# wjqkkky/TTS

Measured on AMD Instinct MI355X. Metric: mel-frames/s (Tacotron2-DDC + MB-MelGAN end-to-end), higher is better.
Workload: dtype f32; 1 GPU; C2: Tacotron2-DDC (r_init=7, r=2, sigmoid attn) + MB-MelGAN [8,4,2]x4, 32 LJ-length utterances per GPU; global_batch=32, r=2, parallelism=replicas x1

## Files before the change

tts_amd/csrc/api_core.hip:

```cpp
#include "host.h"
#include "split16.h"
#include "switches.h"

#include <cmath>
#include <cstring>
#include <memory>

static thread_local std::string g_err;
void tts_set_error(const std::string& m) { g_err = m; }

namespace ttsh {

__global__ void put_rows_kernel(int* dst, RowInts r, int n) {
  if ((int)threadIdx.x < n) dst[threadIdx.x] = r.v[threadIdx.x];
}

const int* put_rows(int* dst, const int32_t* h, int n, hipStream_t s) {
  for (int o = 0; o < n; o += BMAX) {
    const int m = std::min(BMAX, n - o);
    put_rows_kernel<<<1, BMAX, 0, s>>>(dst + o, row_ints(h + o, m), m);
    HIP_OK(hipGetLastError());
  }
  return dst;
}
// ... 155 lines not shown
  a.resid = c.resid;
  a.rb = c.rb;
  a.rc = c.rc;
  a.rt = c.rt;
  a.resid_rows = c.resid_rows;
  a.aux = c.aux;
  a.auxb = c.auxb;
  a.max_q = c.max_q;
  a.B = c.B;
  a.merged_u = c.merged_u;
  TTS_CHECK(!c.merged_u || (c.oflow && L.W16.p), "phase-merged ConvTranspose runs on split-f16 weights only");
  if (c.oflow && L.W16.p && c.nsrc == 1 && (c.s[0].sc != 1 || c.s[0].st % 4 == 0)) {
    a.W16 = L.W16.p;
    a.w16_phase_stride = L.w16_stride;
    a.oflow = c.oflow;
    launch_conv_x3(a, st);
    return;
  }
  launch_conv(a, L.tile, st);
}

void enter(tts_ctx* c, void* stream, bool join_voc) {
  if (c->sv_live && join_voc) {
    HIP_OK(hipStreamWaitEvent(c->s, c->ev_sv, 0));
    c->sv_live = false;
  }
  if (hipStreamQuery((hipStream_t)stream) == hipSuccess) return;
  (void)hipGetLastError();
  HIP_OK(hipEventRecord(c->ev_in, (hipStream_t)stream));
  HIP_OK(hipStreamWaitEvent(c->s, c->ev_in, 0));
}
// ... 151 lines not shown
```

tts_amd/csrc/api_ge2e.hip:

```cpp
#include "host.h"
#include "gsync.h"
#include "split16.h"
#include "switches.h"

#include <cmath>

using namespace ttsh;

namespace {

__global__ void pad_channels_kernel(const float* __restrict__ x, int D, int Dp, long n_rows, float* __restrict__ y) {
  for (long i = (long)blockIdx.x * blockDim.x + threadIdx.x; i < n_rows * Dp; i += (long)gridDim.x * blockDim.x) {
    const long r = i / Dp;
    const int c = (int)(i - r * Dp);
    y[i] = c < D ? x[r * D + c] : 0.f;
  }
}

__global__ __launch_bounds__(256) void ge2e_final_kernel(const float* __restrict__ src, long sb, int width,
                                                         const int* lens, int T_max, const float* __restrict__ W,
                                                         const float* __restrict__ bias, int P,
                                                         float* __restrict__ out) {
  __shared__ float v[1024], red[4];
  const int b = blockIdx.x, tid = threadIdx.x;
// ... 112 lines not shown
  hipStream_t s = c->s;
  const int H = G.H;
  ensure<float>(W.x, (size_t)B * T_max * G.in_pad);
  ensure<int>(W.lens, 64);
  ensure<float>(W.g, (size_t)B * T_max * 4 * H);
  ensure<float>(W.o, (size_t)B * T_max * H);
  ensure<float>(W.p, (size_t)B * T_max * G.proj);
  ensure<unsigned>(W.bar, BAR_WORDS);
  ensure<float>(W.hbuf, (size_t)2 * 64 * H);
  const int* dl = put_rows(W.lens, h_lens, B, s);
  pad_channels_kernel<<<1024, 256, 0, s>>>(d_x, G.in_dim, G.in_pad, (long)B * T_max, W.x.f());
  HIP_OK(hipGetLastError());
  const float* in = W.x.f();
  int din = G.in_pad;
  auto gates = [&](int l) {
    run_conv(G.gin[l], conv_call(c, dl, B, T_max).in(in, btc(T_max, din), din).to(W.g.f(), btc(T_max, 4 * H)), s);
  };
  auto project = [&](int l) {
    run_conv(G.proj_l[l], conv_call(c, dl, B, T_max).in(W.o.f(), btc(T_max, H), H).to(W.p.f(), btc(T_max, G.proj)), s);
  };
  const bool pipe_env = sw::ge2e_pipe();
  bool piped = false;
  if (pipe_env && c->gemm_x3 && G.pipe_ok && B <= 16) {
    gates(0);
    const uint16_t* w16[4] = {nullptr, nullptr, nullptr, nullptr};
    const float* bias[4] = {nullptr, nullptr, nullptr, nullptr};
    for (int l = 0; l < G.nl; ++l) {
      w16[l] = l == 0 ? G.whh16[0].h() : G.wpipe[l].h();
      bias[l] = l == 0 ? nullptr : G.bpipe[l].f();
    }
    piped = launch_ge2e_pipe(w16, bias, G.nl, W.g.f(), dl, T_max, B, W.hbuf.f(), reinterpret_cast<unsigned*>(W.bar.p),
                             W.o.f(), s);
    if (piped && G.with_proj) project(G.nl - 1);
  }
// ... 53 lines not shown
```

tts_amd/csrc/api_glow.hip:

```cpp
#include "host.h"

#include <cmath>
#include <cstdlib>

using namespace ttsh;

namespace {

std::pair<std::vector<float>, std::vector<float>> interleave_halves(const std::vector<float>& w,
                                                                           const std::vector<float>& b, int half,
                                                                           int rowlen) {
  std::vector<float> wo(w.size()), bo(b.size());
  for (int r = 0; r < 2 * half; ++r) {
    const int src = (r & 1) ? half + r / 2 : r / 2;
    std::copy(w.begin() + (size_t)src * rowlen, w.begin() + (size_t)(src + 1) * rowlen, wo.begin() + (size_t)r * rowlen);
    bo[r] = b[src];
  }
  return {wo, bo};
}

void glow_finalize(tts_ctx* c, int num_chars, int enc_layers, int flows, int wn_layers) {
  auto& G = c->glow;
  const auto& h = c->glow_host;
  G.ready = false;
// ... 284 lines not shown
    ensure<float>(W.g, (size_t)B * G.c_pad);
    ensure<float>(W.gcond, (size_t)B * NC);
    if (!W.ones.p) {
      std::vector<int> one(64, 1);
      W.ones.upload(one);
    }
    launch_glow_speaker(put_rows(W.spk, h_spk, B, s), G.emb_g.f(), G.c_in, G.c_pad, W.g.f(), B, s);
    run_conv(G.cond, conv_call(c, W.ones.i(), B, 1).in(W.g.f(), bct(G.c_pad, 1), G.c_pad).to(W.gcond.f(), bct(NC, 1)), s);
  }
  float* x = W.xa.f();
  float* x2 = W.xb.f();
  launch_glow_embed(d_ids, T, G.emb.f(), G.num_chars, H, dl, x, B, s);
  auto conv = [&](const ConvLayer& L, const float* in, int cin, float* out, int cout, int epi,
                  const float* resid = nullptr) {
    ConvCall cc = conv_call(c, dl, B, T).in(in, bct(cin, T), cin).to(out, bct(cout, T)).add(resid, bct(cout, T));
    cc.epi = epi;
    run_conv(L, cc, s);
  };
  if (G.tdsep || G.tfm) {
    float* h0 = W.h2.f();
    float* h1 = W.hdp.f();
    conv(G.pre_conv[0], x, H, h0, H, 0);
    launch_ln(h0, (long)H * T, H, G.pre_g[0].f(), G.pre_b[0].f(), dl, B, T, s, true);
    conv(G.pre_conv[1], h0, H, h1, H, 0);
    launch_ln(h1, (long)H * T, H, G.pre_g[1].f(), G.pre_b[1].f(), dl, B, T, s, true);
    conv(G.pre_conv[2], h1, H, h0, H, 0);
    launch_ln(h0, (long)H * T, H, G.pre_g[2].f(), G.pre_b[2].f(), dl, B, T, s, true);
    conv(G.pre_proj, h0, H, x2, H, 0, x);
    std::swap(x, x2);
    for (int i = 0; i < (G.tfm ? G.enc_layers : 0); ++i) {
// ... 33 lines not shown
  conv(G.dp2, W.hdp.f(), F, W.h2.f(), F, 1);
  launch_ln(W.h2.f(), (long)F * T, F, G.dp_g2.f(), G.dp_b2.f(), dl, B, T, s);
  conv(G.dp_proj, W.h2.f(), F, W.logw.f(), 1, 0);
  launch_glow_durations(W.logw.f(), T, dl, length_scale, W.cum.f(), W.ylens.i(), W.wceil.f(), B, s);
  HIP_OK(hipMemcpyAsync(h_ylens, W.ylens.p, B * 4, hipMemcpyDeviceToHost, s));
  HIP_OK(hipStreamSynchronize(s));
  int mx = 1;
  W.h_ylens.assign(h_ylens, h_ylens + B);
  for (int b = 0; b < B; ++b) mx = std::max(mx, (int)h_ylens[b]);
  W.Ty = mx;
}

struct FlowConvs {
  tts_ctx* c;
  const int* kl;
  int B, K;
  void conv(const ConvLayer& L, const float* in, int in_rows, float* out, int out_rows, const float* resid, int epi,
            int resid_rows = 0, const float* aux = nullptr) const {
    const auto& G = c->glow;
    ConvCall cc = conv_call(c, kl, B, K).in(in, bct(in_rows, K), L.Cin).to(out, bct(out_rows, K));
    cc.add(resid, bct(out_rows, K));
    cc.epi = epi;
    cc.resid_rows = resid_rows;
    cc.aux = aux;
    cc.auxb = (long)G.flows * G.wn_layers * 2 * G.H;
    run_conv(L, cc, c->s);
  }
  float* wn(int k, const float* x) const {
    const auto& G = c->glow;
    auto& W = c->glws;
    const int H = G.H;
    float* hid = W.whs.f();
    float* skip = W.whs.f() + (size_t)H * K;
    conv(G.start[k], x, 2 * G.C, hid, 2 * H, nullptr, 0);
    for (int i = 0; i < G.wn_layers; ++i) {
      const int li = k * G.wn_layers + i;
// ... 15 lines not shown
  const int K1 = std::max(K, 1);
  ensure<float>(W.z, (size_t)B * C * Ty);
  ensure<float>(W.sq, (size_t)B * C2 * K1);
  ensure<float>(W.sq2, (size_t)B * C2 * K1);
  ensure<float>(W.whs, (size_t)B * 2 * H * K1);
  ensure<float>(W.wacts, (size_t)B * H * K1);
  launch_glow_expand(W.om.f(), C, Tx, W.lens.i(), W.cum.f(), W.ylens.i(), Ty, d_noise, noise_scale, d_ymean, W.z.f(),
                     d_attn, B, s);
  HIP_OK(hipMemcpyAsync(d_logw, W.logw.p, (size_t)B * Tx * 4, hipMemcpyDeviceToDevice, s));
  HIP_OK(hipMemsetAsync(d_y, 0, (size_t)B * C * 2 * K * 4, s));
  if (K == 0) return;
  RowInts hk{};
  for (int b = 0; b < B; ++b) hk.v[b] = W.h_ylens[b] / 2;
  const int* kl = put_rows(W.klens, hk.v, B, s);
  launch_glow_squeeze(W.z.f(), C, Ty, W.ylens.i(), W.sq.f(), K, B, s);
  const FlowConvs fc{c, kl, B, K};
  float* x = W.sq.f();
  float* x2 = W.sq2.f();
  for (int k = G.flows - 1; k >= 0; --k) {
    const float* skip = fc.wn(k, x);
    fc.conv(G.end[k], skip, 2 * H, x2, C2, x, 5, 0, G.invtab[k].f());
    std::swap(x, x2);
  }
  launch_glow_unsqueeze(x, C2, K, W.ylens.i(), d_y, 2 * K, B, s);
  HIP_OK(hipStreamSynchronize(s));
}

void glow_search(tts_ctx* c, const float* d_logp, const int* xl, const int* yl, int max_xlen, int B, int Tx, int Ty) {
  auto& W = c->glws;
  ensure<unsigned long long>(W.masbits, (size_t)B * glow_mas_bits_words(Tx, Ty));
  ensure<int>(W.xof, (size_t)B * Ty);
// ... 26 lines not shown
  ensure<int>(W.aylens, 64);
  ensure<int>(W.aklens, 64);
  ensure<float>(W.sq, (size_t)B * C2 * K);
  ensure<float>(W.sq2, (size_t)B * C2 * K);
  ensure<float>(W.eo, (size_t)B * C2 * K);
  ensure<float>(W.whs, (size_t)B * 2 * H * K);
  ensure<float>(W.wacts, (size_t)B * H * K);
  ensure<double>(W.ldpart, (size_t)G.flows * B * tiles);
  if (!d_logp) {
    ensure<float>(W.logp, (size_t)B * Tx * Te);
    d_logp = W.logp.f();
  }
  const int* yl = put_rows(W.aylens, ye2.v, B, s);
  const int* kl = put_rows(W.aklens, ke.v, B, s);
  launch_glow_squeeze(d_y, C, Ty, yl, W.sq.f(), K, B, s);
  const FlowConvs fc{c, kl, B, K};
  float* x = W.sq.f();
  float* x2 = W.sq2.f();
  launch_glow_fwd_glue(x, nullptr, G.fwdtab[0].f(), x2, C, K, kl, nullptr, B, s);
  std::swap(x, x2);
  for (int k = 0; k < G.flows; ++k) {
    const float* skip = fc.wn(k, x);
    fc.conv(G.end[k], skip, 2 * H, W.eo.f(), C2, nullptr, 0);
    launch_glow_fwd_glue(x, W.eo.f(), k + 1 < G.flows ? G.fwdtab[k + 1].f() : nullptr, x2, C, K, kl,
                         static_cast<double*>(W.ldpart.p) + (size_t)k * B * tiles, B, s);
    std::swap(x, x2);
  }
  launch_glow_unsqueeze(x, C2, K, yl, d_z, Te, B, s);
  launch_glow_logdet(static_cast<const double*>(W.ldpart.p), G.flows, tiles, B, kl, G.fwd_logdet_frame, d_logdet, s);
  launch_glow_logp(W.om.f(), C, Tx, W.lens.i(), d_z, Te, yl, d_logp, B, s);
  glow_search(c, d_logp, W.lens.i(), yl, max_xlen, B, Tx, Te);
// ... 79 lines not shown
```

tts_amd/csrc/api_melgan.hip:

```cpp
#include "host.h"
#include "split16.h"
#include "switches.h"

#include <cmath>
#include <cstring>

using namespace ttsh;

static void melgan_finalize(tts_ctx* c, int in_ch, int out_ch, int base, const int32_t* ups, int n_up, int nres,
                     int use_pqmf) {
  auto& G = c->mg;
  const auto& m = c->mg_host;
  G.ready = false;
  TTS_CHECK(nres >= 1 && nres <= 4, "num_res_blocks must be in [1, 4] (dilation <= 27)");
  G.in_ch = in_ch;
  G.out_ch = out_ch;
  G.base = base;
  G.nres = nres;
  G.pqmf = use_pqmf;
  G.ups.assign(ups, ups + n_up);
  G.convT.clear();
  G.dconv.clear();
  G.fused.clear();
  G.convT.resize(n_up);
// ... 109 lines not shown
namespace {

struct GenRun {
  tts_ctx* c;
  const VocCall& v;
  hipStream_t s;
  const int* lens;
  unsigned* oflow;
  int Lb, pad;
  float *x, *xo;
  int C, mul;
  long Ls;
  ConvCall conv(int max_q) const {
    ConvCall cc;
    cc.lens = lens;
    cc.B = v.B;
    cc.max_q = max_q;
    cc.oflow = oflow;
    cc.len_add = 2 * pad;
    return cc;
  }
  void wrote(int C_, long Ls_, int mul_) {
    std::swap(x, xo);
    C = C_;
    Ls = Ls_;
    mul = mul_;
  }
};

GenRun gen_begin(tts_ctx* c, const VocCall& v) {
// ... 286 lines not shown
```

tts_amd/csrc/api_taco.hip:

```cpp
#include "host.h"
#include "decoder.h"
#include "gsync.h"
#include "split16.h"
#include "switches.h"

#include <cstdio>

using namespace ttsh;

DecCtlBlock* ttsh::ctl_block(const TacoWS& W) { return static_cast<DecCtlBlock*>(W.ctl.p); }

DecDev ttsh::make_dev(tts_ctx* c, int Bact) {
  auto& W = c->tws;
  DecDev d{};
  DecCtlBlock* cb = ctl_block(W);
  d.ctl = &cb->ctl;
  d.done = cb->done;
  d.steps = cb->steps;
  d.status = cb->status;
  d.max_steps = cb->max_steps;
  d.lens = W.lens.i();
  d.dec_out = W.dec.f();
  d.align_out = W.align.f();
  d.stop_out = W.stop.f();
// ... 33 lines not shown
    }
  }
  if (q > 0) {
#pragma unroll
    for (int m = 0; m < MB; ++m) red[q - 1][m][c] = acc[m];
  }
  __syncthreads();
  if (q != 0 || n >= N) return;
  const float base = n >= pj0 ? pjb[n - pj0] : 0.f;
#pragma unroll
  for (int m = 0; m < MB; ++m)
    if (m < Bp) out[(long)m * N + n] = base + (m < B ? ((acc[m] + red[0][m][c]) + red[1][m][c]) + red[2][m][c] : 0.f);
  for (int m = MB; m < Bp; ++m) out[(long)m * N + n] = base;
}

void run_encoder(tts_ctx* c, const int64_t* ids, int B, int T_max, float* enc_out, hipStream_t s,
                 const int* rowmap = nullptr) {
  auto& M = c->taco;
  auto& W = c->tws;
  const int* lens = W.lens.i();
  launch_embed_gather(ids, T_max, M.emb.f(), M.num_chars, 512, lens, B, W.x0.f(), s, rowmap);
  const Layout x512 = bct(512, T_max);
  auto conv = [&](const ConvLayer& L, const float* in, Layout li, float* out, Layout lo, int epi) {
    ConvCall cc = conv_call(c, lens, B, T_max).in(in, li, 512).to(out, lo);
    cc.epi = epi;
    run_conv(L, cc, s);
  };
  conv(M.enc[0], W.x0.f(), btc(T_max, 512), W.ca.f(), x512, 1);
  conv(M.enc[1], W.ca.f(), x512, W.cb.f(), x512, 1);
  conv(M.enc[2], W.cb.f(), x512, W.ca.f(), x512, 1);
  conv(M.lstm_in, W.ca.f(), x512, W.gin.f(), btc(T_max, 2048), 0);
  W.enc_ndom = sw::encoder_steps()
                   ? 0
                   : launch_bilstm_persist(W.gin.f(), M.whhT.f(), c->gemm_x3 ? M.whhT16.h() : nullptr, lens, T_max, B,
                                           W.lh.f(), reinterpret_cast<unsigned*>(W.lc.p), enc_out, s);
  W.enc_persist = W.enc_ndom > 0;
  if (!W.enc_persist) {
    HIP_OK(hipMemsetAsync(enc_out, 0, (size_t)B * T_max * 512 * 4, s));
    launch_bilstm(W.gin.f(), M.whhT.f(), lens, T_max, B, W.lh.f(), W.lc.f(), enc_out, s);
// ... 5 lines not shown
    "TTS_BARRIER_TIMEOUT_MS; retrying the call is safe)";
bool all_zero(const int* p, int n) {
  return std::all_of(p, p + n, [](int w) { return w == 0; });
}
void check_encoder_barrier(tts_ctx* c) {
  if (!c->tws.enc_persist) return;
  int* pw = c->pinned + PIN_ENC;
  const int nd = std::min(c->tws.enc_ndom, ENC_NDOM_MAX);
  std::fill(pw, pw + ENC_NDOM_MAX, 0);
  const unsigned* words = reinterpret_cast<const unsigned*>(c->tws.lc.p);
  for (int i = 0; i < nd; ++i) HIP_OK(hipMemcpyAsync(&pw[i], words + i * BAR_WORDS + 16, 4, hipMemcpyDeviceToHost, c->s));
  HIP_OK(hipStreamSynchronize(c->s));
  TTS_CHECK(all_zero(pw, ENC_NDOM_MAX), ENC_BAR_MSG);
}

void run_postnet(tts_ctx* c, const float* dec, long dec_b, const int* mlens, int B, int Mmax_alloc, int max_q,
                 float* out, long out_b, hipStream_t s) {
  auto& M = c->taco;
  auto& W = c->tws;
  const Layout x512 = bct(512, Mmax_alloc), frames{dec_b, 1, 80};
  auto conv = [&](const ConvLayer& L, const float* in, Layout li, int Cin, float* o, Layout lo, int epi,
                  const float* resid) {
    ConvCall cc = conv_call(c, mlens, B, max_q).in(in, li, Cin).to(o, lo);
    if (resid) cc.add(resid, frames);
    cc.epi = epi;
    run_conv(L, cc, s);
  };
  conv(M.post[0], dec, frames, 80, W.pa.f(), x512, 2, nullptr);
  float* bufs[2] = {W.pa.f(), W.pbb.f()};
  for (int i = 1; i < 4; ++i) conv(M.post[i], bufs[(i - 1) & 1], x512, 512, bufs[i & 1], x512, 2, nullptr);
  conv(M.post[4], bufs[1], x512, 512, out, Layout{out_b, 1, 80}, 0, dec);
}

template <class T>
__global__ void gather_rows_kernel(const T* __restrict__ src, T* __restrict__ dst, const int* __restrict__ map,
                                   long row) {
  const long i = blockIdx.y;
  const T* sr = src + (long)map[i] * row;
// ... 359 lines not shown
                               "per call on a 256-CU device)");
  if (d_spk_emb) {
    gather_rows<float>(d_spk_emb, spk_out, W.map.i(), M.es, B, s);
  } else {
    TTS_CHECK(M.num_spk > 0, "model has no speaker_embedding table: pass speaker embeddings");
    gather_rows<int64_t>(d_spk_ids, reinterpret_cast<int64_t*>(W.spkid.p), W.map.i(), 1, B, s);
    launch_embed_gather(reinterpret_cast<const int64_t*>(W.spkid.p), 1, M.spk_table.f(), M.num_spk, M.es,
                        W.lens.i(), B, spk_out, s);
  }
  if (M.gst_dim) {
    gst_cond_kernel<<<B, 256, 0, s>>>(d_style, W.map.i(), spk_out, M.gst_dim, M.es, W.spk.f());
    HIP_OK(hipGetLastError());
  }
}

void run_encoder_penc(tts_ctx* c, const int64_t* ids, int B, int T_max, hipStream_t s) {
  auto& W = c->tws;
  run_encoder(c, ids, B, T_max, W.enc.f(), s, W.map.i());
  run_conv(c->taco.penc,
           conv_call(c, W.lens.i(), B, T_max).in(W.enc.f(), btc(T_max, 512), 512).to(W.penc.f(), btc(T_max, 128)), s);
}

void fill_decoder_state(tts_ctx* c, int B, int T_max, int S_cap, int r, bool persist, hipStream_t s) {
  auto& M = c->taco;
  auto& W = c->tws;
  const int Bp = W.MT * 16;
  FillList f;
  for (const DevBuf* b : {&W.catt, &W.hatt, &W.hdec0, &W.hdec1, &W.cdec}) f.add(b->p, (size_t)Bp * 1024 * 4);
  f.add(W.ctx.p, (size_t)Bp * 512 * 4);
  f.add(W.y.p, (size_t)Bp * 80 * M.r_init * 4);
  f.add(W.alpha.p, (size_t)B * T_max * 4);
  f.add(W.acum.p, (size_t)B * T_max * 4);
  f.add(W.dec.p, (size_t)B * S_cap * r * 80 * 4);
  f.add(W.align.p, (size_t)B * S_cap * T_max * 4);
  f.add(W.stop.p, (size_t)B * S_cap * 4);
// ... 2 lines not shown
  if (persist)
    for (int li = 0; li < W.MT; ++li) add_barrier_fills(f, reinterpret_cast<unsigned*>(W.pbar.p) + BAR_WORDS * W.pslot[li], 1);
  launch_fills(f, s);
  bcast_rows_kernel<<<256, 256, 0, s>>>(M.att_bias.f(), 4096, W.gatt.f(), Bp);
  HIP_OK(hipGetLastError());
}


void run_postnet_scatter(tts_ctx* c, int B, int T_max, int S_cap, int r, float* d_dec, float* d_post, float* d_align,
                         float* d_stop, hipStream_t s, const RowInts* ml = nullptr) {
  auto& W = c->tws;
  taco_mlens_kernel<<<1, 64, 0, s>>>(ctl_block(W), B, r, W.mlens.i());
  HIP_OK(hipGetLastError());
  const long fb = (long)S_cap * r * 80;
  if (ml) mask_frames(W.dec.f(), *ml, W.mlens.i(), B, r, fb, s);
  run_postnet(c, W.dec.f(), fb, W.mlens.i(), B, S_cap * r, S_cap * r, W.post.f(), fb, s);
  if (ml) mask_frames(W.post.f(), *ml, W.mlens.i(), B, r, fb, s);
  gather4_rows(Gather4{{W.post.f(), W.dec.f(), W.align.f(), W.stop.f()}, {d_post, d_dec, d_align, d_stop},
                       {fb, fb, (long)S_cap * T_max, (long)S_cap}},
               W.map.i() + BMAX, B, s);
}

void read_status(tts_ctx* c, int B, int r, bool persist, const FusedVoc* fv, hipStream_t s) {
  auto& W = c->tws;
  const unsigned* lc = reinterpret_cast<const unsigned*>(W.lc.p);
  DecSlots ds;
  std::copy(W.pslot, W.pslot + PMAX_LAUNCH, ds.v);
  taco_status_kernel<<<1, 256, 0, s>>>(W.enc_persist ? lc : nullptr, W.enc_ndom,
                                       persist ? reinterpret_cast<const unsigned*>(W.pbar.p) : nullptr, ds,
                                       c->dec_nlaunch, ctl_block(W), c->gemm_x3 ? x3_flag(c) : nullptr, W.stat.i(), B,
                                       W.map.i() + BMAX, r, fv ? fv->Lmin : 0, fv ? fv->vlens : nullptr);
// ... 56 lines not shown
  const int max_ms = check_infer_args(M, k.h_lens, B, T_max, r, h_max_steps, S_cap);
  taco_workspace(c, B, T_max, S_cap, r);
  auto& W = c->tws;
  if (t) grow<float>(W.teach, (size_t)S_cap * W.MT * 16 * 256, W.gen);
  hipStream_t s = c->s;
  enter(c, k.stream, !fv);
  const std::vector<int> perm = stage_decode_order(c, k.h_lens, h_max_steps, B, fv ? x3_flag(c) : nullptr, s);
  W.thr = t ? 0.5f : k.run.thr;
  const bool persist = use_persistent(c);
  TTS_CHECK(!t || persist, "teacher-forced forward runs on the persistent decoder only (<= 64 utterances per "
                           "call on a 256-CU device, TTS_DECODER=graph unset)");
  TTS_CHECK(!M.variant() || persist, "BN prenet / attention windowing / forward / Graves attention run on "
                                     "the persistent decoder only (<= 64 utterances per call on a 256-CU "
                                     "device)");
  stage_speakers(c, k.d_spk_ids, k.d_spk_emb, k.d_style, B, s);
  run_encoder_penc(c, k.ids, B, T_max, s);
  if (persist && !W.pslot_cal) {
    pick_barrier_blocks(reinterpret_cast<unsigned*>(W.pbar.p), PBAR_CAND, PMAX_LAUNCH, W.pslot, s);
    W.pslot_cal = true;
  }
  fill_decoder_state(c, B, T_max, S_cap, r, persist, s);
  RowInts ml{};
  if (t) {
    TeachArgs ta{};
    ta.mel = t->d_mel;
    ta.mel_b = (long)t->M_max * 80;
    ta.map = W.map.i();
    ta.max_steps = ctl_block(W)->max_steps;
    ta.W1 = M.pre1.f();
    ta.b1 = M.prenet_bn ? M.pre1_b0.f() : nullptr;
    ta.teach = W.teach.f();
// ... 80 lines not shown
    with_x3_fallback(c, [&] { taco_run(c, k); });
  });
}

int tts_taco_encoder(tts_ctx* c, const int64_t* d_ids, const int32_t* h_lens, int B, int T_max, float* d_out,
                     void* stream) {
  return guarded_ctx(c, [&] {
    TTS_CHECK(c && d_ids && h_lens && d_out, "null argument");
    TTS_CHECK(c->taco.ready, "tacotron2 weights not finalized");
    TTS_CHECK(B >= 1 && B <= BMAX && T_max >= 1, "bad sizes");
    check_rows(h_lens, B, 1, T_max, "lens out of range");
    DeviceGuard g(c->device);
    taco_workspace(c, B, T_max, std::max(1, c->tws.S_cap), std::max(1, c->tws.r));
    enter(c, stream);
    put_rows(c->tws.lens, h_lens, B, c->s);
    with_x3_fallback(c, [&] { run_encoder(c, d_ids, B, T_max, d_out, c->s); });
    check_encoder_barrier(c);
    leave(c, stream);
  });
}

int tts_taco_postnet(tts_ctx* c, const float* d_dec, const int32_t* h_lens, int B, int M_max, float* d_out,
                     void* stream) {
  return guarded_ctx(c, [&] {
    TTS_CHECK(c && d_dec && h_lens && d_out, "null argument");
    TTS_CHECK(c->taco.ready, "tacotron2 weights not finalized");
    TTS_CHECK(B >= 1 && B <= BMAX && M_max >= 1, "bad sizes");
    DeviceGuard g(c->device);
    auto& W = c->tws;
    long gen = W.gen;
    grow<int>(W.mlens, BMAX, gen);
    grow<float>(W.pa, (size_t)B * 512 * M_max, gen);
    grow<float>(W.pbb, (size_t)B * 512 * M_max, gen);
    W.gen = gen;
    check_rows(h_lens, B, 1, M_max, "lens out of range");
    const int maxM = *std::max_element(h_lens, h_lens + B);
    enter(c, stream);
    put_rows(W.mlens, h_lens, B, c->s);
    HIP_OK(hipMemsetAsync(d_out, 0, (size_t)B * M_max * 80 * 4, c->s));
    with_x3_fallback(c, [&] {
      run_postnet(c, d_dec, (long)M_max * 80, W.mlens.i(), B, M_max, maxM, d_out, (long)M_max * 80, c->s);
    });
    HIP_OK(hipStreamSynchronize(c->s));
    leave(c, stream);
  });
}

int tts_taco_decoder_state(tts_ctx* c, int B, int T_max, float* d_att_h, float* d_att_c, float* d_dec_h,
                           float* d_dec_c, float* d_context, float* d_alpha, float* d_alpha_cum, void* stream) {
  return guarded_ctx(c, [&] {
    TTS_CHECK(c->last_B > 0, "run tts_taco_infer first");
    TTS_CHECK(B == c->last_B && T_max == c->last_T,
              "decoder state: the buffers' (B, T_max) differ from the last decode on this context");
    TTS_CHECK(c->dec_path == 1 && c->dec_nlaunch >= 1, "decoder state: the last decode did not run the persistent "
                                                       "decoder (TTS_DECODER=graph or a non-256-CU device)");
    DeviceGuard g(c->device);
// ... 32 lines not shown
```

tts_amd/csrc/common.h:

```cpp
#pragma once
#include <hip/hip_runtime.h>
#include <atomic>
#include <cstdint>
#include <mutex>
#include <set>
#include <string>
#include <tuple>
#include <vector>

typedef float f32x4 __attribute__((ext_vector_type(4)));

constexpr int BMAX = 64;

struct RowInts {
  int v[BMAX];
};

#define MFMA16(a, b, c) __builtin_amdgcn_mfma_f32_16x16x4f32((a), (b), (c), 0, 0, 0)

void tts_set_error(const std::string& msg);

#define HIP_OK(expr)                                                                   \
  do {                                                                                 \
    hipError_t _e = (expr);                                                            \
// ... 88 lines not shown
  const float* aux;
  long auxb;
  int max_q;
  int B;
  const void* W16 = nullptr;
  long w16_phase_stride = 0;
  unsigned* oflow = nullptr;
  int merged_u = 0;
};

enum ConvTile { TILE_128x64 = 0, TILE_64x64, TILE_192x64, TILE_96x64, TILE_48x128, TILE_80x64, TILE_16x256 };
int conv_tile_tc(int tile);
int conv_tile_for_cout(int cout);
void launch_conv(const ConvArgs& a, int tile, hipStream_t s);
bool conv_x3_supported(int Cin, int Cout, int K, int dil);
void launch_conv_x3(const ConvArgs& a, hipStream_t s);
std::vector<uint16_t> pack_conv_x3(const std::vector<float>& Wm, int Cin, int Cout, int K, int nphase,
                                   long* phase_stride_bytes);
std::vector<float> merge_convT_phases(const std::vector<float>& Wm, int u, int Cin, int Cout);

void swizzle_rows16(const float* Wm, int rows, int rows_pad, int Kdim, float* dst);

struct FillList {
  static constexpr int N = 32;
  int n = 0;
  void* p[N];
  long words[N];
  unsigned val[N];
  void add(void* ptr, size_t bytes, unsigned v = 0) {
    TTS_CHECK(n < N && bytes % 4 == 0, "FillList: too many entries or unaligned size");
    if (!bytes) return;
// ... 68 lines not shown
```

tts_amd/csrc/conv_x3.hip:

```cpp
#include "common.h"
#include "conv_epi.h"
#include "split16.h"
#include "switches.h"
#include "x3_tile.h"

#include <algorithm>
#include <mutex>
#include <map>

namespace {
constexpr int CX_XR = 80;
}

template <int MI, int NI, int WM, int WN, int KT, int RS, int SD>
__global__ __launch_bounds__(64 * WM * WN) void conv_x3_kernel(ConvArgs a, int nq, int nco, int nz) {
  constexpr int NTHR = 64 * WM * WN;
  constexpr int TC = 16 * MI * WM, TQ = 16 * NI * WN;
  constexpr int SPT = (4 * (TQ + CONV_MAX_SPAN) + NTHR - 1) / NTHR;
  static_assert(RS == KT || RS == 2 * KT, "weight ring: one or two chunks of taps");
  extern __shared__ __attribute__((aligned(16))) _Float16 shx[];

  const int ntile = nq * nco * nz;
  const int per = (ntile + 7) / 8;
  const int w = (int)(blockIdx.x % 8) * per + (int)(blockIdx.x / 8);
  if (w >= ntile) return;
  const int cot = w / (nq * nz);
  const int rem = w - cot * nq * nz;
  const int z = rem / nq;
  const int qt = rem - z * nq;

  const int ph = z % a.nphase;
  const int b = z / a.nphase;
  const int base = a.lens[b] + a.len_add;
  const int Lq = base * a.q_mul + (a.merged_u ? 1 : 0);
  const int q0 = qt * TQ;
  if (q0 >= Lq) return;
  const int co0 = cot * TC;
  const int Lin = base * a.in_mul;
  const int dil = a.dil;
  const int span = (KT - 1) * dil;
  const int ROWS = TQ + span;
  _Float16* X0 = shx;
  _Float16* X1 = shx + ROWS * CX_XR;

  const int tid = threadIdx.x;
  const int lane = tid & 63, wave = __builtin_amdgcn_readfirstlane(tid >> 6);
  const int wm = wave / WN, wn = wave % WN;
  const int nb = wn * 16 * NI + (lane & 15);
  const int kg = 8 * (lane >> 4);
  const int NCH = (a.Cin + 31) / 32;
  const int NKS = NCH * KT;
  const int mtiles = (a.Cout + 15) / 16;
  bool bad = false;

  const ConvSrc& S = a.src[0];
  const int i0 = q0 - a.pad_left[ph];
  const bool interior = (a.rep_pad == 0) && i0 >= 0 && i0 + ROWS <= Lin;
  const int rawL = a.lens[b];
  const int Lsrc = a.rep_pad ? rawL : Lin;
  const bool tmajor = S.sc == 1;
  const __amdgpu_buffer_rsrc_t xr = __builtin_amdgcn_make_buffer_rsrc(
      const_cast<float*>(S.ptr + (long)b * S.sb), 0,
      (int)min((long)0x7fffffff, ((long)(S.C - 1) * S.sc + (long)(Lsrc - 1) * S.st + 1) * 4), 0x00020000);
  int voff[SPT], sgv[SPT], srow[SPT];
  bool sval[SPT];
#pragma unroll
  for (int j = 0; j < SPT; ++j) {
    const int e = tid + NTHR * j;
    const int g = e / ROWS;
    srow[j] = e - g * ROWS;
    sgv[j] = g;
    int i = i0 + srow[j];
    bool valid = true;
// ... 210 lines not shown
  if (Cout == 192) return CX_T192;
  if (Cout == 96) return CX_T96;
  if (Cout == 80) return CX_T80;
  if (Cout == 48) return CX_T48;
  if (Cout % 64 == 0) return CX_T64;
  if (Cout % 80 == 0) return CX_T80;
  return CX_NONE;
}

bool conv_x3_supported(int Cin, int Cout, int K, int dil) {
  return Cin % 8 == 0 && Cin >= 8 && cx_tile(Cout) != CX_NONE && (K == 1 || K == 2 || K == 3 || K == 5 || K == 7) &&
         (K - 1) * dil <= CONV_MAX_SPAN;
}

template <int MI, int NI, int WM, int WN, int KT, int RS, int SD>
static void cx_launch(const ConvArgs& a, hipStream_t s) {
  constexpr int TC = 16 * MI * WM, TQ = 16 * NI * WN;
  ensure_dyn_lds((const void*)conv_x3_kernel<MI, NI, WM, WN, KT, RS, SD>, 160 * 1024);
  const int nq = (a.max_q + TQ - 1) / TQ, nco = (a.Cout + TC - 1) / TC, nz = a.B * a.nphase;
  const long ntile = (long)nq * nco * nz;
  TTS_CHECK(ntile < (1L << 30), "conv_x3: grid too large");
  const int per = (int)((ntile + 7) / 8);
  const size_t lds = (size_t)2 * (TQ + (KT - 1) * a.dil) * CX_XR * 2;
  conv_x3_kernel<MI, NI, WM, WN, KT, RS, SD><<<dim3(8 * per), 64 * WM * WN, lds, s>>>(a, nq, nco, nz);
}

template <int MI, int NI, int WM, int WN, int KT, int RS, int SD>
static long cx_cost_k(const ConvArgs& a) {
  constexpr int TC = 16 * MI * WM, TQ = 16 * NI * WN;
  const void* f = (const void*)conv_x3_kernel<MI, NI, WM, WN, KT, RS, SD>;
  const size_t lds = (size_t)2 * (TQ + (KT - 1) * a.dil) * CX_XR * 2;
  static std::mutex mu;
  static std::map<size_t, long> slots_by_lds;
  long slots;
  ensure_dyn_lds(f, 160 * 1024);
  const int cus = device_cu_count();
  {
    std::lock_guard<std::mutex> lk(mu);
    auto it = slots_by_lds.find(lds);
    if (it == slots_by_lds.end()) {
      int nb = 0;
      HIP_OK(hipOccupancyMaxActiveBlocksPerMultiprocessor(&nb, f, 64 * WM * WN, lds));
      it = slots_by_lds.emplace(lds, std::max(1L, (long)nb * cus)).first;
    }
    slots = it->second;
  }
// ... 1 lines not shown
  return (tiles + slots - 1) / slots * TQ;
}
template <int MI, int NI, int WM, int WN, int SD12>
static long cx_cost(const ConvArgs& a) {
  switch (a.K) {
    case 1: return cx_cost_k<MI, NI, WM, WN, 1, 2, SD12>(a);
    case 2: return cx_cost_k<MI, NI, WM, WN, 2, 2 * SD12, SD12>(a);
    case 3: return cx_cost_k<MI, NI, WM, WN, 3, 3, 1>(a);
    case 5: return cx_cost_k<MI, NI, WM, WN, 5, 5, 2>(a);
    case 7: return cx_cost_k<MI, NI, WM, WN, 7, 7, 1>(a);
    default: return 0;
  }
}

template <int MI, int NI, int WM, int WN, int SD12>
static void cx_taps(const ConvArgs& a, hipStream_t s) {
  switch (a.K) {
    case 1: cx_launch<MI, NI, WM, WN, 1, 2, SD12>(a, s); break;
    case 2: cx_launch<MI, NI, WM, WN, 2, 2 * SD12, SD12>(a, s); break;
    case 3: cx_launch<MI, NI, WM, WN, 3, 3, 1>(a, s); break;
    case 5: cx_launch<MI, NI, WM, WN, 5, 5, 2>(a, s); break;
    case 7: cx_launch<MI, NI, WM, WN, 7, 7, 1>(a, s); break;
    default: TTS_CHECK(false, "conv_x3: unsupported tap count");
  }
}

void launch_conv_x3(const ConvArgs& a, hipStream_t s) {
  TTS_CHECK(conv_x3_supported(a.Cin, a.Cout, a.K, a.dil), "conv_x3: unsupported shape");
  TTS_CHECK(a.W16 && a.oflow, "conv_x3: split weights / overflow flag missing");
  TTS_CHECK(a.nphase >= 1 && a.nphase <= 8, "conv: nphase");
  TTS_CHECK(a.nsrc == 1 && a.src[0].C == a.Cin, "conv_x3: one source");
  TTS_CHECK(!a.merged_u || (a.nphase == 1 && a.K == 2 && a.pad_left[0] == 1 && a.pad_mode == 0 && a.epi_act == 0 &&
                            a.rep_pad == 0 && a.Cout % a.merged_u == 0 && a.merged_u % 2 == 0),
            "conv_x3: phase-merged ConvTranspose arguments");
  TTS_CHECK(a.src[0].sc != 1 || (a.src[0].st % 4 == 0 && (reinterpret_cast<uintptr_t>(a.src[0].ptr) & 15) == 0),
            "conv_x3: time-major source rows must be 16-byte aligned");
  if (a.max_q <= 0 || a.B <= 0) return;
  switch (cx_tile(a.Cout)) {
    case CX_T128: {
      const int force = sw::cx_ni128();
      bool narrow = force == 3;
      if (!force && a.K >= 2) narrow = cx_cost<2, 3, 4, 1, 2>(a) < cx_cost<2, 4, 4, 1, 2>(a);
      if (narrow) cx_taps<2, 3, 4, 1, 2>(a, s);
      else cx_taps<2, 4, 4, 1, 2>(a, s);
      break;
    }
    case CX_T192: cx_taps<3, 4, 4, 1, 2>(a, s); break;
    case CX_T96: cx_taps<3, 4, 2, 2, 1>(a, s); break;
    case CX_T64: cx_taps<2, 4, 2, 2, 1>(a, s); break;
    case CX_T80: cx_taps<5, 2, 1, 4, 2>(a, s); break;
    case CX_T48: cx_taps<3, 2, 1, 4, 1>(a, s); break;
    default: TTS_CHECK(false, "conv_x3: unsupported output channel count");
  }
  HIP_OK(hipGetLastError());
}

std::vector<uint16_t> pack_conv_x3(const std::vector<float>& Wm, int Cin, int Cout, int K, int nphase,
                                   long* phase_stride_bytes) {
  const int nch = (Cin + 31) / 32, mtiles = (Cout + 15) / 16;
  const size_t per = (size_t)mtiles * nch * K * 64 * 16;
  std::vector<uint16_t> out(per * nphase);
  for (int ph = 0; ph < nphase; ++ph) {
    const float* w = Wm.data() + (size_t)ph * Cout * Cin * K;
    auto blk = pack_split_a(mtiles, nch * K, [&](int m, int k) -> float {
      const int step = k / 32, ch = step / K, tap = step % K, ci = 32 * ch + k % 32;
      return (m < Cout && ci < Cin) ? w[((size_t)m * Cin + ci) * K + tap] : 0.f;
// ... 15 lines not shown
```

tts_amd/csrc/host.h:

```cpp
#pragma once
#include "common.h"
#include "launch.h"
#include "../../include/ttship.h"

#include <algorithm>
#include <functional>
#include <map>
#include <mutex>
#include <stdexcept>
#include <string>
#include <vector>

struct DecCtlBlock;
struct DecDev;

namespace ttsh {

constexpr int CHUNK = 8;

struct DevBuf {
  void* p = nullptr;
  size_t bytes = 0;
  DevBuf() = default;
  DevBuf(const DevBuf&) = delete;
// ... 74 lines not shown
  long b;
  int c, t;
};
inline Layout bct(int C, long T) { return {(long)C * T, (int)T, 1}; }
inline Layout btc(long T, int C) { return {T * C, 1, C}; }

struct ConvCall {
  ConvCall& in(const float* p, Layout l, int C, int act = 0) { return s[0] = ConvSrc{p, l.b, l.c, l.t, C, act}, *this; }
  ConvCall& in2(const float* p, Layout l, int C) { return s[1] = ConvSrc{p, l.b, l.c, l.t, C, 0}, nsrc = 2, *this; }
  ConvCall& to(float* p, Layout l) { return out = p, ob = l.b, oc = l.c, ot = l.t, *this; }
  ConvCall& add(const float* p, Layout l) { return resid = p, rb = l.b, rc = l.c, rt = l.t, *this; }
  ConvSrc s[2];
  int nsrc = 1;
  int pad_mode = 0;
  const int* lens = nullptr;
  int len_add = 0, in_mul = 1, q_mul = 1, rep_pad = 0, out_mul = 1;
  float* out = nullptr;
  long ob = 0;
  int oc = 0, ot = 0;
  int epi = 0;
  const float* resid = nullptr;
  long rb = 0;
  int rc = 0, rt = 0, resid_rows = 0;
  const float* aux = nullptr;
  long auxb = 0;
  int max_q = 0, B = 0;
  unsigned* oflow = nullptr;
  int merged_u = 0;
};

// ... 433 lines not shown
```

tts_amd/csrc/switches.h:

```cpp
#pragma once
#include <cstdlib>
#include <string>

namespace sw {

inline bool on_unless_zero(const char* name, bool dflt) {
  const char* e = std::getenv(name);
  return e ? std::atoi(e) != 0 : dflt;
}
inline bool on_unless_one(const char* name) {
  const char* e = std::getenv(name);
  return !e || std::atoi(e) != 1;
}
inline bool present(const char* name) { return std::getenv(name) != nullptr; }
inline int number(const char* name, int dflt) {
  const char* e = std::getenv(name);
  return e ? std::atoi(e) : dflt;
}
inline std::string text(const char* name) {
  const char* e = std::getenv(name);
  return e ? e : "";
}

inline bool gemm_f32() { static const bool v = text("TTS_GEMM") == "f32"; return v; }
// ... 16 lines not shown
inline bool decoder_graph() { static const bool v = text("TTS_DECODER") == "graph"; return v; }
inline bool decoder_f32() { static const bool v = present("TTS_DECODER_F32"); return v; }
inline bool align_in_p4() { static const bool v = present("TTS_ALIGN_IN_P4"); return v; }
inline const char* ptrace_file() {
  static const bool set = present("TTS_PTRACE");
  static const std::string v = text("TTS_PTRACE");
  return set ? v.c_str() : nullptr;
}
inline int ptrace_t0() { static const int v = number("TTS_PTRACE_T0", 100); return v; }
inline int ptrace_launch() { static const int v = number("TTS_PTRACE_LAUNCH", 0); return v; }

inline bool stack_fuse() { static const bool v = on_unless_zero("TTS_STACK_FUSE", true); return v; }
inline bool stack_fuse96() { static const bool v = on_unless_zero("TTS_STACK_FUSE96", false); return v; }
inline bool ct_fuse() { static const bool v = on_unless_zero("TTS_CT_FUSE", true); return v; }
inline int cx_ni128() { static const int v = number("TTS_CX_NI128", 0); return v; }

inline bool ge2e_pipe() { static const bool v = text("TTS_GE2E_PIPE") != "0"; return v; }

inline int pwgan_staging() {
  static const int v = [] {
    const std::string e = text("TTS_PWGAN_STAGING");
    return e == "regs" ? 0 : e == "ring4" ? 2 : 1;
  }();
  return v;
}
inline int pwgan_tile() { static const int v = number("TTS_PWGAN_TILE", 0); return v; }

}
```

Measured before the change: 1.335 million mel-frames/s.

## Deal conv_x3 tiles over ragged per-utterance lengths instead of padded grid

The split-f16 conv kernel gets a ragged scheduling mode. Each block prefix-sums per-row tile counts in LDS and maps its block index onto only the tiles that fall inside each utterance's real length. Where host lengths are available, the grid is shrunk to the real tile count, so fewer blocks launch only to exit early on padded positions. Host length pointers are threaded through every conv call site to make this possible. The cost is extra LDS and a wave-level scan at kernel start. The cx_ragged switch is not cached, so it calls getenv on every launch.

After: 1.329 million mel-frames/s. About the same (-0.4%).

```diff
diff --git a/tts_amd/csrc/api_core.hip b/tts_amd/csrc/api_core.hip
--- a/tts_amd/csrc/api_core.hip
+++ b/tts_amd/csrc/api_core.hip
@@ -193,7 +193,7 @@
     a.W16 = L.W16.p;
     a.w16_phase_stride = L.w16_stride;
     a.oflow = c.oflow;
-    launch_conv_x3(a, st);
+    launch_conv_x3(a, c.h_lens, st);
     return;
   }
   launch_conv(a, L.tile, st);
diff --git a/tts_amd/csrc/api_ge2e.hip b/tts_amd/csrc/api_ge2e.hip
--- a/tts_amd/csrc/api_ge2e.hip
+++ b/tts_amd/csrc/api_ge2e.hip
@@ -150,10 +150,14 @@
   const float* in = W.x.f();
   int din = G.in_pad;
   auto gates = [&](int l) {
-    run_conv(G.gin[l], conv_call(c, dl, B, T_max).in(in, btc(T_max, din), din).to(W.g.f(), btc(T_max, 4 * H)), s);
+    ConvCall cc = conv_call(c, dl, B, T_max).in(in, btc(T_max, din), din).to(W.g.f(), btc(T_max, 4 * H));
+    cc.h_lens = h_lens;
+    run_conv(G.gin[l], cc, s);
   };
   auto project = [&](int l) {
-    run_conv(G.proj_l[l], conv_call(c, dl, B, T_max).in(W.o.f(), btc(T_max, H), H).to(W.p.f(), btc(T_max, G.proj)), s);
+    ConvCall cc = conv_call(c, dl, B, T_max).in(W.o.f(), btc(T_max, H), H).to(W.p.f(), btc(T_max, G.proj));
+    cc.h_lens = h_lens;
+    run_conv(G.proj_l[l], cc, s);
   };
   const bool pipe_env = sw::ge2e_pipe();
   bool piped = false;
diff --git a/tts_amd/csrc/api_glow.hip b/tts_amd/csrc/api_glow.hip
--- a/tts_amd/csrc/api_glow.hip
+++ b/tts_amd/csrc/api_glow.hip
@@ -322,6 +322,7 @@
   auto conv = [&](const ConvLayer& L, const float* in, int cin, float* out, int cout, int epi,
                   const float* resid = nullptr) {
     ConvCall cc = conv_call(c, dl, B, T).in(in, bct(cin, T), cin).to(out, bct(cout, T)).add(resid, bct(cout, T));
+    cc.h_lens = h_lens;
     cc.epi = epi;
     run_conv(L, cc, s);
   };
@@ -385,12 +386,14 @@
 struct FlowConvs {
   tts_ctx* c;
   const int* kl;
+  const int32_t* h_kl;
   int B, K;
   void conv(const ConvLayer& L, const float* in, int in_rows, float* out, int out_rows, const float* resid, int epi,
             int resid_rows = 0, const float* aux = nullptr) const {
     const auto& G = c->glow;
     ConvCall cc = conv_call(c, kl, B, K).in(in, bct(in_rows, K), L.Cin).to(out, bct(out_rows, K));
     cc.add(resid, bct(out_rows, K));
+    cc.h_lens = h_kl;
     cc.epi = epi;
     cc.resid_rows = resid_rows;
     cc.aux = aux;
@@ -436,7 +439,7 @@
   for (int b = 0; b < B; ++b) hk.v[b] = W.h_ylens[b] / 2;
   const int* kl = put_rows(W.klens, hk.v, B, s);
   launch_glow_squeeze(W.z.f(), C, Ty, W.ylens.i(), W.sq.f(), K, B, s);
-  const FlowConvs fc{c, kl, B, K};
+  const FlowConvs fc{c, kl, hk.v, B, K};
   float* x = W.sq.f();
   float* x2 = W.sq2.f();
   for (int k = G.flows - 1; k >= 0; --k) {
@@ -493,7 +496,7 @@
   const int* yl = put_rows(W.aylens, ye2.v, B, s);
   const int* kl = put_rows(W.aklens, ke.v, B, s);
   launch_glow_squeeze(d_y, C, Ty, yl, W.sq.f(), K, B, s);
-  const FlowConvs fc{c, kl, B, K};
+  const FlowConvs fc{c, kl, ke.v, B, K};
   float* x = W.sq.f();
   float* x2 = W.sq2.f();
   launch_glow_fwd_glue(x, nullptr, G.fwdtab[0].f(), x2, C, K, kl, nullptr, B, s);
diff --git a/tts_amd/csrc/api_melgan.hip b/tts_amd/csrc/api_melgan.hip
--- a/tts_amd/csrc/api_melgan.hip
+++ b/tts_amd/csrc/api_melgan.hip
@@ -147,6 +147,7 @@
   ConvCall conv(int max_q) const {
     ConvCall cc;
     cc.lens = lens;
+    cc.h_lens = v.h_lens;
     cc.B = v.B;
     cc.max_q = max_q;
     cc.oflow = oflow;
diff --git a/tts_amd/csrc/api_taco.hip b/tts_amd/csrc/api_taco.hip
--- a/tts_amd/csrc/api_taco.hip
+++ b/tts_amd/csrc/api_taco.hip
@@ -71,8 +71,8 @@
   for (int m = MB; m < Bp; ++m) out[(long)m * N + n] = base;
 }
 
-void run_encoder(tts_ctx* c, const int64_t* ids, int B, int T_max, float* enc_out, hipStream_t s,
-                 const int* rowmap = nullptr) {
+void run_encoder(tts_ctx* c, const int64_t* ids, const int32_t* h_lens, int B, int T_max, float* enc_out,
+                 hipStream_t s, const int* rowmap = nullptr) {
   auto& M = c->taco;
   auto& W = c->tws;
   const int* lens = W.lens.i();
@@ -80,6 +80,7 @@
   const Layout x512 = bct(512, T_max);
   auto conv = [&](const ConvLayer& L, const float* in, Layout li, float* out, Layout lo, int epi) {
     ConvCall cc = conv_call(c, lens, B, T_max).in(in, li, 512).to(out, lo);
+    cc.h_lens = h_lens;
     cc.epi = epi;
     run_conv(L, cc, s);
   };
@@ -115,14 +116,15 @@
   TTS_CHECK(all_zero(pw, ENC_NDOM_MAX), ENC_BAR_MSG);
 }
 
-void run_postnet(tts_ctx* c, const float* dec, long dec_b, const int* mlens, int B, int Mmax_alloc, int max_q,
-                 float* out, long out_b, hipStream_t s) {
+void run_postnet(tts_ctx* c, const float* dec, long dec_b, const int* mlens, const int32_t* h_mlens, int B,
+                 int Mmax_alloc, int max_q, float* out, long out_b, hipStream_t s) {
   auto& M = c->taco;
   auto& W = c->tws;
   const Layout x512 = bct(512, Mmax_alloc), frames{dec_b, 1, 80};
   auto conv = [&](const ConvLayer& L, const float* in, Layout li, int Cin, float* o, Layout lo, int epi,
                   const float* resid) {
     ConvCall cc = conv_call(c, mlens, B, max_q).in(in, li, Cin).to(o, lo);
+    cc.h_lens = h_mlens;
     if (resid) cc.add(resid, frames);
     cc.epi = epi;
     run_conv(L, cc, s);
@@ -512,11 +514,12 @@
   }
 }
 
-void run_encoder_penc(tts_ctx* c, const int64_t* ids, int B, int T_max, hipStream_t s) {
-  auto& W = c->tws;
-  run_encoder(c, ids, B, T_max, W.enc.f(), s, W.map.i());
-  run_conv(c->taco.penc,
-           conv_call(c, W.lens.i(), B, T_max).in(W.enc.f(), btc(T_max, 512), 512).to(W.penc.f(), btc(T_max, 128)), s);
+void run_encoder_penc(tts_ctx* c, const int64_t* ids, const int32_t* h_lens, int B, int T_max, hipStream_t s) {
+  auto& W = c->tws;
+  run_encoder(c, ids, h_lens, B, T_max, W.enc.f(), s, W.map.i());
+  ConvCall cc = conv_call(c, W.lens.i(), B, T_max).in(W.enc.f(), btc(T_max, 512), 512).to(W.penc.f(), btc(T_max, 128));
+  cc.h_lens = h_lens;
+  run_conv(c->taco.penc, cc, s);
 }
 
 void fill_decoder_state(tts_ctx* c, int B, int T_max, int S_cap, int r, bool persist, hipStream_t s) {
@@ -549,7 +552,7 @@
   HIP_OK(hipGetLastError());
   const long fb = (long)S_cap * r * 80;
   if (ml) mask_frames(W.dec.f(), *ml, W.mlens.i(), B, r, fb, s);
-  run_postnet(c, W.dec.f(), fb, W.mlens.i(), B, S_cap * r, S_cap * r, W.post.f(), fb, s);
+  run_postnet(c, W.dec.f(), fb, W.mlens.i(), nullptr, B, S_cap * r, S_cap * r, W.post.f(), fb, s);
   if (ml) mask_frames(W.post.f(), *ml, W.mlens.i(), B, r, fb, s);
   gather4_rows(Gather4{{W.post.f(), W.dec.f(), W.align.f(), W.stop.f()}, {d_post, d_dec, d_align, d_stop},
                        {fb, fb, (long)S_cap * T_max, (long)S_cap}},
@@ -636,7 +639,7 @@
                                      "the persistent decoder only (<= 64 utterances per call on a 256-CU "
                                      "device)");
   stage_speakers(c, k.d_spk_ids, k.d_spk_emb, k.d_style, B, s);
-  run_encoder_penc(c, k.ids, B, T_max, s);
+  run_encoder_penc(c, k.ids, k.h_lens, B, T_max, s);
   if (persist && !W.pslot_cal) {
     pick_barrier_blocks(reinterpret_cast<unsigned*>(W.pbar.p), PBAR_CAND, PMAX_LAUNCH, W.pslot, s);
     W.pslot_cal = true;
@@ -747,7 +750,7 @@
     taco_workspace(c, B, T_max, std::max(1, c->tws.S_cap), std::max(1, c->tws.r));
     enter(c, stream);
     put_rows(c->tws.lens, h_lens, B, c->s);
-    with_x3_fallback(c, [&] { run_encoder(c, d_ids, B, T_max, d_out, c->s); });
+    with_x3_fallback(c, [&] { run_encoder(c, d_ids, h_lens, B, T_max, d_out, c->s); });
     check_encoder_barrier(c);
     leave(c, stream);
   });
@@ -772,7 +775,7 @@
     put_rows(W.mlens, h_lens, B, c->s);
     HIP_OK(hipMemsetAsync(d_out, 0, (size_t)B * M_max * 80 * 4, c->s));
     with_x3_fallback(c, [&] {
-      run_postnet(c, d_dec, (long)M_max * 80, W.mlens.i(), B, M_max, maxM, d_out, (long)M_max * 80, c->s);
+      run_postnet(c, d_dec, (long)M_max * 80, W.mlens.i(), h_lens, B, M_max, maxM, d_out, (long)M_max * 80, c->s);
     });
     HIP_OK(hipStreamSynchronize(c->s));
     leave(c, stream);
diff --git a/tts_amd/csrc/common.h b/tts_amd/csrc/common.h
--- a/tts_amd/csrc/common.h
+++ b/tts_amd/csrc/common.h
@@ -126,7 +126,7 @@
 int conv_tile_for_cout(int cout);
 void launch_conv(const ConvArgs& a, int tile, hipStream_t s);
 bool conv_x3_supported(int Cin, int Cout, int K, int dil);
-void launch_conv_x3(const ConvArgs& a, hipStream_t s);
+void launch_conv_x3(const ConvArgs& a, const int* h_lens, hipStream_t s);
 std::vector<uint16_t> pack_conv_x3(const std::vector<float>& Wm, int Cin, int Cout, int K, int nphase,
                                    long* phase_stride_bytes);
 std::vector<float> merge_convT_phases(const std::vector<float>& Wm, int u, int Cin, int Cout);
diff --git a/tts_amd/csrc/conv_x3.hip b/tts_amd/csrc/conv_x3.hip
--- a/tts_amd/csrc/conv_x3.hip
+++ b/tts_amd/csrc/conv_x3.hip
@@ -1,5 +1,6 @@
 #include "common.h"
 #include "conv_epi.h"
+#include "cx_deal.h"
 #include "split16.h"
 #include "switches.h"
 #include "x3_tile.h"
@@ -10,6 +11,9 @@
 
 namespace {
 constexpr int CX_XR = 80;
+constexpr size_t cx_lds_bytes(int TQ, int KT, int dil) {
+  return (size_t)2 * (TQ + (KT - 1) * dil) * CX_XR * 2 + (2 * CX_DEAL_ROWS + 1 + 3) / 4 * 16;
+}
 }
 
 template <int MI, int NI, int WM, int WN, int KT, int RS, int SD>
@@ -19,19 +23,51 @@
   constexpr int SPT = (4 * (TQ + CONV_MAX_SPAN) + NTHR - 1) / NTHR;
   static_assert(RS == KT || RS == 2 * KT, "weight ring: one or two chunks of taps");
   extern __shared__ __attribute__((aligned(16))) _Float16 shx[];
-
-  const int ntile = nq * nco * nz;
-  const int per = (ntile + 7) / 8;
-  const int w = (int)(blockIdx.x % 8) * per + (int)(blockIdx.x / 8);
-  if (w >= ntile) return;
-  const int cot = w / (nq * nz);
-  const int rem = w - cot * nq * nz;
-  const int z = rem / nq;
-  const int qt = rem - z * nq;
-
-  const int ph = z % a.nphase;
-  const int b = z / a.nphase;
-  const int base = a.lens[b] + a.len_add;
+  int* tcum = reinterpret_cast<int*>(shx + 2 * (TQ + (KT - 1) * a.dil) * CX_XR);
+
+  int cot, b, ph, qt, rawL;
+  if (nq == 0) {
+    if (threadIdx.x < 64) {
+      const int lane = threadIdx.x;
+      const int len = lane < a.B ? a.lens[lane] : 0;
+      const int n = lane < a.B ? cx_row_tiles(len, a.len_add, a.q_mul, a.merged_u, a.max_q, a.nphase, TQ) : 0;
+      int v = n;
+#pragma unroll
+      for (int o = 1; o < 64; o <<= 1) {
+        const int y = __shfl_up(v, o, 64);
+        if (lane >= o) v += y;
+      }
+      tcum[lane] = v - n;
+      tcum[CX_DEAL_ROWS + 1 + lane] = len;
+      if (lane == 63) tcum[64] = v;
+    }
+    lds_barrier();
+    const int rowsum = tcum[64];
+    const int w = __builtin_amdgcn_readfirstlane(cx_deal_entry((int)blockIdx.x, rowsum, nco));
+    if (w < 0) return;
+    const int r = w % rowsum;
+    const unsigned long long m = __ballot(cx_row_hit(tcum, a.B, (int)(threadIdx.x & 63), r));
+    const int row = __builtin_amdgcn_readfirstlane(m ? __ffsll((long long)m) - 1 : 0);
+    const CxTile t = cx_tile_in_row(tcum, w, rowsum, row, a.nphase);
+    cot = __builtin_amdgcn_readfirstlane(t.cot);
+    b = row;
+    rawL = __builtin_amdgcn_readfirstlane(tcum[CX_DEAL_ROWS + 1 + row]);
+    ph = __builtin_amdgcn_readfirstlane(t.ph);
+    qt = __builtin_amdgcn_readfirstlane(t.qt);
+  } else {
+    const int ntile = nq * nco * nz;
+    const int per = (ntile + 7) / 8;
+    const int w = (int)(blockIdx.x % 8) * per + (int)(blockIdx.x / 8);
+    if (w >= ntile) return;
+    cot = w / (nq * nz);
+    const int rem = w - cot * nq * nz;
+    const int z = rem / nq;
+    qt = rem - z * nq;
+    ph = z % a.nphase;
+    b = z / a.nphase;
+    rawL = a.lens[b];
+  }
+  const int base = rawL + a.len_add;
   const int Lq = base * a.q_mul + (a.merged_u ? 1 : 0);
   const int q0 = qt * TQ;
   if (q0 >= Lq) return;
@@ -56,7 +92,6 @@
   const ConvSrc& S = a.src[0];
   const int i0 = q0 - a.pad_left[ph];
   const bool interior = (a.rep_pad == 0) && i0 >= 0 && i0 + ROWS <= Lin;
-  const int rawL = a.lens[b];
   const int Lsrc = a.rep_pad ? rawL : Lin;
   const bool tmajor = S.sc == 1;
   const __amdgpu_buffer_rsrc_t xr = __builtin_amdgcn_make_buffer_rsrc(
@@ -297,22 +332,29 @@
 }
 
 template <int MI, int NI, int WM, int WN, int KT, int RS, int SD>
-static void cx_launch(const ConvArgs& a, hipStream_t s) {
+static void cx_launch(const ConvArgs& a, const int* h_lens, hipStream_t s) {
   constexpr int TC = 16 * MI * WM, TQ = 16 * NI * WN;
   ensure_dyn_lds((const void*)conv_x3_kernel<MI, NI, WM, WN, KT, RS, SD>, 160 * 1024);
   const int nq = (a.max_q + TQ - 1) / TQ, nco = (a.Cout + TC - 1) / TC, nz = a.B * a.nphase;
-  const long ntile = (long)nq * nco * nz;
+  long ntile = (long)nq * nco * nz;
   TTS_CHECK(ntile < (1L << 30), "conv_x3: grid too large");
+  bool ragged = a.B > 1 && a.B <= CX_DEAL_ROWS && sw::cx_ragged();
+  if (ragged && h_lens) {
+    const long real = cx_rowsum_host(h_lens, a.B, a.len_add, a.q_mul, a.merged_u, a.max_q, a.nphase, TQ) * nco;
+    if (real == ntile) ragged = false;
+    ntile = std::min(ntile, real);
+  }
+  if (ntile <= 0) return;
   const int per = (int)((ntile + 7) / 8);
-  const size_t lds = (size_t)2 * (TQ + (KT - 1) * a.dil) * CX_XR * 2;
-  conv_x3_kernel<MI, NI, WM, WN, KT, RS, SD><<<dim3(8 * per), 64 * WM * WN, lds, s>>>(a, nq, nco, nz);
+  const size_t lds = cx_lds_bytes(TQ, KT, a.dil);
+  conv_x3_kernel<MI, NI, WM, WN, KT, RS, SD><<<dim3(8 * per), 64 * WM * WN, lds, s>>>(a, ragged ? 0 : nq, nco, nz);
 }
 
 template <int MI, int NI, int WM, int WN, int KT, int RS, int SD>
 static long cx_cost_k(const ConvArgs& a) {
   constexpr int TC = 16 * MI * WM, TQ = 16 * NI * WN;
   const void* f = (const void*)conv_x3_kernel<MI, NI, WM, WN, KT, RS, SD>;
-  const size_t lds = (size_t)2 * (TQ + (KT - 1) * a.dil) * CX_XR * 2;
+  const size_t lds = cx_lds_bytes(TQ, KT, a.dil);
   static std::mutex mu;
   static std::map<size_t, long> slots_by_lds;
   long slots;
@@ -344,18 +386,18 @@
 }
 
 template <int MI, int NI, int WM, int WN, int SD12>
-static void cx_taps(const ConvArgs& a, hipStream_t s) {
+static void cx_taps(const ConvArgs& a, const int* h_lens, hipStream_t s) {
   switch (a.K) {
-    case 1: cx_launch<MI, NI, WM, WN, 1, 2, SD12>(a, s); break;
-    case 2: cx_launch<MI, NI, WM, WN, 2, 2 * SD12, SD12>(a, s); break;
-    case 3: cx_launch<MI, NI, WM, WN, 3, 3, 1>(a, s); break;
-    case 5: cx_launch<MI, NI, WM, WN, 5, 5, 2>(a, s); break;
-    case 7: cx_launch<MI, NI, WM, WN, 7, 7, 1>(a, s); break;
+    case 1: cx_launch<MI, NI, WM, WN, 1, 2, SD12>(a, h_lens, s); break;
+    case 2: cx_launch<MI, NI, WM, WN, 2, 2 * SD12, SD12>(a, h_lens, s); break;
+    case 3: cx_launch<MI, NI, WM, WN, 3, 3, 1>(a, h_lens, s); break;
+    case 5: cx_launch<MI, NI, WM, WN, 5, 5, 2>(a, h_lens, s); break;
+    case 7: cx_launch<MI, NI, WM, WN, 7, 7, 1>(a, h_lens, s); break;
     default: TTS_CHECK(false, "conv_x3: unsupported tap count");
   }
 }
 
-void launch_conv_x3(const ConvArgs& a, hipStream_t s) {
+void launch_conv_x3(const ConvArgs& a, const int* h_lens, hipStream_t s) {
   TTS_CHECK(conv_x3_supported(a.Cin, a.Cout, a.K, a.dil), "conv_x3: unsupported shape");
   TTS_CHECK(a.W16 && a.oflow, "conv_x3: split weights / overflow flag missing");
   TTS_CHECK(a.nphase >= 1 && a.nphase <= 8, "conv: nphase");
@@ -371,15 +413,15 @@
       const int force = sw::cx_ni128();
       bool narrow = force == 3;
       if (!force && a.K >= 2) narrow = cx_cost<2, 3, 4, 1, 2>(a) < cx_cost<2, 4, 4, 1, 2>(a);
-      if (narrow) cx_taps<2, 3, 4, 1, 2>(a, s);
-      else cx_taps<2, 4, 4, 1, 2>(a, s);
+      if (narrow) cx_taps<2, 3, 4, 1, 2>(a, h_lens, s);
+      else cx_taps<2, 4, 4, 1, 2>(a, h_lens, s);
       break;
     }
-    case CX_T192: cx_taps<3, 4, 4, 1, 2>(a, s); break;
-    case CX_T96: cx_taps<3, 4, 2, 2, 1>(a, s); break;
-    case CX_T64: cx_taps<2, 4, 2, 2, 1>(a, s); break;
-    case CX_T80: cx_taps<5, 2, 1, 4, 2>(a, s); break;
-    case CX_T48: cx_taps<3, 2, 1, 4, 1>(a, s); break;
+    case CX_T192: cx_taps<3, 4, 4, 1, 2>(a, h_lens, s); break;
+    case CX_T96: cx_taps<3, 4, 2, 2, 1>(a, h_lens, s); break;
+    case CX_T64: cx_taps<2, 4, 2, 2, 1>(a, h_lens, s); break;
+    case CX_T80: cx_taps<5, 2, 1, 4, 2>(a, h_lens, s); break;
+    case CX_T48: cx_taps<3, 2, 1, 4, 1>(a, h_lens, s); break;
     default: TTS_CHECK(false, "conv_x3: unsupported output channel count");
   }
   HIP_OK(hipGetLastError());
diff --git a/tts_amd/csrc/cx_deal.h b/tts_amd/csrc/cx_deal.h
--- /dev/null
+++ b/tts_amd/csrc/cx_deal.h
@@ -0,0 +1,48 @@
+#pragma once
+
+#if defined(__HIPCC__)
+#define CX_HD __host__ __device__ __forceinline__
+#else
+#define CX_HD inline
+#endif
+
+constexpr int CX_DEAL_ROWS = 64;
+
+CX_HD int cx_row_tiles(int len, int len_add, int q_mul, int merged_u, int max_q, int nphase, int TQ) {
+  int Lq = (len + len_add) * q_mul + (merged_u ? 1 : 0);
+  Lq = Lq < max_q ? Lq : max_q;
+  return Lq > 0 ? (Lq + TQ - 1) / TQ * nphase : 0;
+}
+
+CX_HD int cx_deal_entry(int p, int rowsum, int nco) {
+  const int total = rowsum * nco;
+  const int q = total / 8, rem = total - 8 * q;
+  const int x = p % 8, slot = p / 8;
+  const int run = q + (x < rem ? 1 : 0);
+  return slot < run ? x * q + (x < rem ? x : rem) + slot : -1;
+}
+
+CX_HD bool cx_row_hit(const int* tcum, int B, int row, int r) {
+  return row < B && tcum[row] <= r && r < tcum[row + 1];
+}
+
+struct CxTile {
+  int cot, b, ph, qt;
+};
+CX_HD CxTile cx_tile_in_row(const int* tcum, int w, int rowsum, int b, int nphase) {
+  CxTile t;
+  t.cot = w / rowsum;
+  const int i = w - t.cot * rowsum - tcum[b];
+  const int n = (tcum[b + 1] - tcum[b]) / nphase;
+  t.b = b;
+  t.ph = i / n;
+  t.qt = i - t.ph * n;
+  return t;
+}
+
+inline long cx_rowsum_host(const int* h_lens, int B, int len_add, int q_mul, int merged_u, int max_q, int nphase,
+                           int TQ) {
+  long s = 0;
+  for (int b = 0; b < B; ++b) s += cx_row_tiles(h_lens[b], len_add, q_mul, merged_u, max_q, nphase, TQ);
+  return s;
+}
diff --git a/tts_amd/csrc/host.h b/tts_amd/csrc/host.h
--- a/tts_amd/csrc/host.h
+++ b/tts_amd/csrc/host.h
@@ -112,6 +112,7 @@
   int nsrc = 1;
   int pad_mode = 0;
   const int* lens = nullptr;
+  const int32_t* h_lens = nullptr;
   int len_add = 0, in_mul = 1, q_mul = 1, rep_pad = 0, out_mul = 1;
   float* out = nullptr;
   long ob = 0;
diff --git a/tts_amd/csrc/switches.h b/tts_amd/csrc/switches.h
--- a/tts_amd/csrc/switches.h
+++ b/tts_amd/csrc/switches.h
@@ -54,6 +54,7 @@
 inline bool stack_fuse96() { static const bool v = on_unless_zero("TTS_STACK_FUSE96", false); return v; }
 inline bool ct_fuse() { static const bool v = on_unless_zero("TTS_CT_FUSE", true); return v; }
 inline int cx_ni128() { static const int v = number("TTS_CX_NI128", 0); return v; }
+inline bool cx_ragged() { return on_unless_zero("TTS_CX_RAGGED", true); }
 
 inline bool ge2e_pipe() { static const bool v = text("TTS_GE2E_PIPE") != "0"; return v; }
 
```
